# jjery2243542/adaptive_voice_conversion

Measured on NVIDIA H100. Metric: mel-segments/sec (80x128) train step, higher is better.
Workload: dtype tf32

## Files before the change

adaptive_voice_conversion_b200/csrc/wgrad_tc.cu:

```cuda
#include "common.cuh"
#include "tc_common.cuh"
#include "tmap.cuh"

namespace avc {

constexpr int WT_NT = 32;
constexpr int WG_ROWS = 32;
constexpr int WG_A_PLANE = 32 * 4 * 16;
constexpr int WG_A_BYTES = (WG_ROWS / 4) * WG_A_PLANE;
constexpr int WG_MAX_STAGES = 8;
constexpr int WG_SMEM_MAX = 224 * 1024;

struct WgTcArgs {
  avc_wgrad_desc d;
  float* scratch;
  int nslices, samp_per_slice, nstage, coutp;
  int* status;
};

__device__ __forceinline__ float comp4(const float4& v, int c) { return c == 0 ? v.x : c == 1 ? v.y : c == 2 ? v.z : v.w; }

struct WgJob {
  float4 v[4];
  uint32_t dst;
  int rot;
};

template <int K>
__device__ __forceinline__ WgJob wgrad_job_load(const WgTcArgs& a, int e, int ch, int b0, int R) {
  const avc_wgrad_desc& d = a.d;
  const int T = d.Tout;
  WgJob J;
  const int c4 = e & 7, pl = (e >> 3) & 7, j = e >> 6;
  const int r = ch * WG_ROWS + 4 * pl;
  const int g = r / T, t = r - g * T;
  J.rot = (c4 >> 1) & 3;
  J.dst = (uint32_t)WG_A_BYTES + (uint32_t)pl * (uint32_t)(K * WT_NT * 16) + (uint32_t)(j * WT_NT + 4 * c4) * 16u;
  const int ci = blockIdx.x * WT_NT + 4 * c4;
  const bool v = r < R && ci < d.Cin;
  const float* col = d.x + (size_t)(v ? b0 + g : 0) * d.x_bstride + (size_t)((v ? ci : 0) >> 2) * d.Tin * 4;
#pragma unroll
  for (int i = 0; i < 4; ++i) {
    const int p = src_pos((t + i) * d.stride + j - d.pad_left, d.Tin, AVC_PAD_REFLECT, 1);
    J.v[i] = (v && p >= 0) ? ldg4(col + (size_t)p * 4) : zero4();
  }
  return J;
}

__device__ __forceinline__ void wgrad_job_store(uint8_t* stage, const WgJob& J) {
#pragma unroll
  for (int k = 0; k < 4; ++k) {
    const int c = (k + J.rot) & 3;
    *reinterpret_cast<float4*>(stage + J.dst + (uint32_t)c * 16u) = make_float4(comp4(J.v[0], c), comp4(J.v[1], c), comp4(J.v[2], c), comp4(J.v[3], c));
  }
}

__host__ __device__ constexpr int wg_stagers(int K) { return K <= 6 ? 2 : 1; }
__host__ __device__ constexpr int wg_threads(int K) { return 128 * (wg_stagers(K) + 2); }
__host__ __device__ constexpr int wg_regs_stage(int K) { return wg_stagers(K) == 2 ? 96 : 104; }
__host__ __device__ constexpr int wg_regs_mma(int K) { return wg_stagers(K) == 2 ? 160 : 200; }
static_assert(2 * 128 * wg_regs_stage(1) + 256 * wg_regs_mma(1) <= 512 * 128 && 128 * wg_regs_stage(8) + 256 * wg_regs_mma(8) <= 384 * 168,
              "setmaxnreg budget exceeds the launch allocation");

template <int N>
__device__ __forceinline__ bool wgrad_mma_stage(const WgTcArgs& a, float* acc, uint32_t* af, uint32_t* af_prev, uint64_t* full, int s, uint32_t ph,
                                                const uint8_t* stage, uint32_t a_off, uint32_t b_lo, uint32_t d_hi) {
  constexpr uint32_t B_PLANE = N * 16;
  if (!__all_sync(0xffffffffu, tc::mbar_wait(&full[s], ph, a.status, 6))) {
    tc::wgmma_wait<0>();
    return false;
  }
#pragma unroll
  for (int k = 0; k < WG_ROWS / 8; ++k)
#pragma unroll
    for (int q = 0; q < 4; ++q)
      af[4 * k + q] = *reinterpret_cast<const uint32_t*>(stage + a_off + (uint32_t)(2 * k + (q >> 1)) * WG_A_PLANE + (uint32_t)(q & 1) * 128u);
  tc::wgmma_fence();
#pragma unroll
  for (int k = 0; k < WG_ROWS / 8; ++k)
    tc::wgmma_tf32_rs<N>(acc, af + 4 * k, tc::sdesc64(b_lo + (uint32_t)k * ((2u * B_PLANE) >> 4), d_hi), 1u);
  tc::wgmma_commit();
  tc::wgmma_wait<1>();
  tc::acc_fence(acc, N / 2);
  tc::reg_fence(af_prev, 16);
  return true;
}

template <int K, bool ATOMIC>
__global__ void __launch_bounds__(wg_threads(K), 1) conv_wgrad_wgmma_kernel(const WgTcArgs a, const __grid_constant__ CUtensorMap tmdc) {
  constexpr int STAGERS = wg_stagers(K);
  constexpr int N = K * WT_NT;
  constexpr uint32_t B_PLANE = N * 16;
  extern __shared__ __align__(1024) uint8_t smem[];
  __shared__ uint64_t bar_full[WG_MAX_STAGES], bar_empty[WG_MAX_STAGES];
  const avc_wgrad_desc& d = a.d;
  const int tid = threadIdx.x, warp = tc::warp_idx_sync(), lane = tid & 31;
  const int sl = blockIdx.z, b0 = sl * a.samp_per_slice;
  const int R = max(0, min(a.samp_per_slice, d.B - b0)) * d.Tout;
  const int nchunk = cdiv(R, WG_ROWS);
  const uint32_t stage_bytes = (uint32_t)WG_A_BYTES + 8u * B_PLANE;

  if (tid == 0) {
    for (int s = 0; s < a.nstage; ++s) {
      tc::mbar_init(&bar_full[s], 5);
      tc::mbar_init(&bar_empty[s], 2);
    }
    tc::fence_mbar_init();
  }
  __syncthreads();

  if (warp < 4 * STAGERS) {
    tc::setmaxnreg_dec<wg_regs_stage(K)>();
    constexpr int NJOBS = 64 * K, JPT = (NJOBS + 127) / 128;
    const int stid = tid & 127;
    for (int ch = warp >> 2; ch < nchunk; ch += STAGERS) {
      const int s = ch % a.nstage;
      const uint32_t ph = (uint32_t)(ch / a.nstage) & 1u;
      WgJob J[JPT];
#pragma unroll
      for (int q = 0; q < JPT; ++q)
        if (stid + 128 * q < NJOBS) J[q] = wgrad_job_load<K>(a, stid + 128 * q, ch, b0, R);
      if (ch >= a.nstage && !__all_sync(0xffffffffu, tc::mbar_wait(&bar_empty[s], ph ^ 1u, a.status, 5))) return;
      uint8_t* stage = smem + (size_t)s * stage_bytes;
      if (stid == 0) {
        tc::mbar_arrive_expect_tx(&bar_full[s], (uint32_t)WG_A_BYTES);
#pragma unroll
        for (int p = 0; p < WG_ROWS / 4; ++p) {
          const int r = ch * WG_ROWS + 4 * p, g = r / d.Tout;
          tc::tensor_g2s_4d(stage + p * WG_A_PLANE, &tmdc, 0, r - g * d.Tout, blockIdx.y * 32, r < R ? b0 + g : d.B, &bar_full[s]);
        }
      }
#pragma unroll
      for (int q = 0; q < JPT; ++q)
        if (stid + 128 * q < NJOBS) wgrad_job_store(stage, J[q]);
      tc::fence_proxy_async_smem();
      __syncwarp();
      if (lane == 0) tc::mbar_arrive(&bar_full[s]);
    }
    return;
  }

  tc::setmaxnreg_inc<wg_regs_mma(K)>();
  const int wg = (warp >> 2) - STAGERS, wt = tid & 127;
  float acc[N / 2];
#pragma unroll
  for (int i = 0; i < N / 2; ++i) acc[i] = 0.f;
  const int m = 64 * wg + tc::wg_acc_row(wt, 0);
  const uint32_t a_off = (uint32_t)(m >> 2) * 64u + (uint32_t)(wt & 3) * 16u + (uint32_t)(m & 3) * 4u;
  uint32_t af[2][16];
  const uint32_t smem0 = tc::smem_u32(smem), d_hi = tc::sdesc_hi(128);
  int s = 0, s_prev = -1;
  uint32_t ph = 0;
  tc::acc_fence(acc, N / 2);
  for (int ch = 0; ch < nchunk; ++ch) {
    const uint32_t b_lo = tc::sdesc_lo(smem0 + (uint32_t)s * stage_bytes + (uint32_t)WG_A_BYTES, B_PLANE);
    const uint8_t* stage = smem + (size_t)s * stage_bytes;
    const bool ok = (ch & 1) ? wgrad_mma_stage<N>(a, acc, af[1], af[0], bar_full, s, ph, stage, a_off, b_lo, d_hi)
                             : wgrad_mma_stage<N>(a, acc, af[0], af[1], bar_full, s, ph, stage, a_off, b_lo, d_hi);
    if (!ok) return;
    if (s_prev >= 0 && wt == 0) tc::mbar_arrive(&bar_empty[s_prev]);
    s_prev = s;
    if (++s == a.nstage) { s = 0; ph ^= 1u; }
  }
  tc::wgmma_wait<0>();
  tc::acc_fence(acc, N / 2);
  tc::reg_fence(af[0], 16);
  tc::reg_fence(af[1], 16);
  if (nchunk == 0) return;

  const int co = blockIdx.y * 128 + m;
#pragma unroll
  for (int jj = 0; jj < N / 8; ++jj) {
    const int n = tc::wg_acc_col(wt, 4 * jj), j = n / WT_NT, ci = blockIdx.x * WT_NT + n % WT_NT;
    if (ci < d.Cin) {
      float* sbase = a.scratch + (((size_t)(ATOMIC ? 0 : sl) * K + j) * (size_t)(d.Cin >> 2)) * (size_t)a.coutp * 4;
#pragma unroll
      for (int h = 0; h < 2; ++h) {
        float* p = sbase + ((size_t)(ci >> 2) * a.coutp + co + 8 * h) * 4 + (ci & 3);
        const float v0 = acc[4 * jj + 2 * h], v1 = acc[4 * jj + 2 * h + 1];
        if constexpr (ATOMIC)
          asm volatile("red.global.add.v2.f32 [%0], {%1, %2};" ::"l"(p), "f"(v0), "f"(v1) : "memory");
        else
          *reinterpret_cast<float2*>(p) = make_float2(v0, v1);
      }
    }
  }
}

__global__ void __launch_bounds__(256) wgrad_tc_reduce_kernel(const float* __restrict__ scratch, float* __restrict__ dw, int Cout, int Cin,
                                                              int K, int coutp, int nslices) {
  __shared__ float4 part[8][32];
  const int64_t n = (int64_t)K * (Cin >> 2) * coutp;
  const int64_t slice_stride = n * 4;
  const int64_t i = (int64_t)blockIdx.x * 32 + threadIdx.x;
  float4 s = zero4();
  if (i < n) {
    int sl = threadIdx.y;
    float4 s1 = zero4();
    const float* p = scratch + i * 4;
    for (; sl + 24 < nslices; sl += 32) {
      const float4 v0 = ldg4(p + (sl + 0) * slice_stride), v1 = ldg4(p + (sl + 8) * slice_stride);
      const float4 v2 = ldg4(p + (sl + 16) * slice_stride), v3 = ldg4(p + (sl + 24) * slice_stride);
      s.x += v0.x + v2.x; s.y += v0.y + v2.y; s.z += v0.z + v2.z; s.w += v0.w + v2.w;
      s1.x += v1.x + v3.x; s1.y += v1.y + v3.y; s1.z += v1.z + v3.z; s1.w += v1.w + v3.w;
    }
    s.x += s1.x; s.y += s1.y; s.z += s1.z; s.w += s1.w;
    for (; sl < nslices; sl += 8) {
      const float4 v = ldg4(scratch + sl * slice_stride + i * 4);
      s.x += v.x; s.y += v.y; s.z += v.z; s.w += v.w;
    }
  }
  part[threadIdx.y][threadIdx.x] = s;
  __syncthreads();
  if (threadIdx.y == 0 && i < n) {
#pragma unroll
    for (int y = 1; y < 8; ++y) { const float4 v = part[y][threadIdx.x]; s.x += v.x; s.y += v.y; s.z += v.z; s.w += v.w; }
    const int co = (int)(i % coutp);
    if (co < Cout) {
      const int64_t r = i / coutp;
      const int c4 = (int)(r % (Cin >> 2)), j = (int)(r / (Cin >> 2));
      float* o = dw + ((int64_t)co * Cin + c4 * 4) * K + j;
      o[0] += s.x; o[K] += s.y; o[2 * K] += s.z; o[3 * K] += s.w;
    }
  }
}

__global__ void __launch_bounds__(256) wgrad_acc_flush_kernel(const avc_wgrad_acc_item* __restrict__ items) {
  __shared__ float tile[32][32 * 8 + 1];
  const avc_wgrad_acc_item it = items[blockIdx.y];
  const int K = it.K, C4 = it.Cin >> 2;
  const int coutp = cdiv(it.Cout, 128) * 128;
  const int ncg = cdiv(C4, 8);
  const int nblk = (coutp >> 5) * ncg;
  if ((int)blockIdx.x >= nblk) return;
  const int cot = blockIdx.x / ncg, cg = blockIdx.x - cot * ncg;
  const int co0 = cot << 5, c40 = cg << 3;
  const int tid = threadIdx.x, col = tid & 31, c4l = tid >> 5;
  if (c40 + c4l < C4) {
    for (int j = 0; j < K; ++j) {
      float4* a4 = reinterpret_cast<float4*>(it.acc) + ((size_t)j * C4 + c40 + c4l) * coutp + co0 + col;
      const float4 s = *a4;
      *a4 = zero4();
      float* t = &tile[col][(c4l * 4) * K + j];
      t[0] = s.x; t[K] = s.y; t[2 * K] = s.z; t[3 * K] = s.w;
    }
  }
  __syncthreads();
  const int nci = min(32, it.Cin - c40 * 4);
  const int run = nci * K;
  for (int r = tid >> 5; r < 32; r += 8) {
    const int co = co0 + r;
    if (co >= it.Cout) break;
    float* o = it.dw + ((size_t)co * it.Cin + c40 * 4) * K;
    for (int e = tid & 31; e < run; e += 32) o[e] += tile[r][e];
  }
}

static int wgrad_tc_plan(const avc_wgrad_desc* d, WgTcArgs& a) {
  const int T = d->Tout;
  a.d = *d;
  int G = T >= 128 ? 1 : 128 / T;
  if (d->stride == 2) G = T >= 64 ? 1 : 64 / T;
  a.coutp = cdiv(d->Cout, 128) * 128;
  const int ntiles = cdiv(d->B, G);
  const int cta_per_slice = cdiv(d->Cin, WT_NT) * cdiv(d->Cout, 128);
  int nsl = 132 / cta_per_slice;
  if (nsl < 1) nsl = 1;
  if (nsl > ntiles) nsl = ntiles;
  const int tiles_per_slice = cdiv(ntiles, nsl);
  a.nslices = cdiv(ntiles, tiles_per_slice);
  a.samp_per_slice = tiles_per_slice * G;
  a.nstage = min(WG_MAX_STAGES, WG_SMEM_MAX / (WG_A_BYTES + 8 * 16 * WT_NT * d->K));
  return AVC_OK;
}

static bool wgrad_tc_supported(const avc_wgrad_desc* d) {
  return (d->stride == 1 || d->stride == 2) && d->Tout % 8 == 0 && d->Tout <= 128 && d->K >= 1 && d->K <= 8 && d->Cin % 4 == 0 &&
         d->Cout % 4 == 0 && d->Tin + d->K - 1 >= (d->Tout - 1) * d->stride + 1 && (d->stride == 1 || d->Tout <= 64);
}

int wgrad_reduce(const float* scratch, float* dw, int Cout, int Cin, int K, int coutp, int nslices, cudaStream_t stream) {
  const int64_t n = (int64_t)K * (Cin / 4) * coutp;
  AVC_LAUNCH(wgrad_tc_reduce_kernel, (int)cdiv64(n, 32), dim3(32, 8), 0, stream, scratch, dw, Cout, Cin, K, coutp, nslices);
  AVC_CHECK_LAUNCH("wgrad_tc_reduce");
  return AVC_OK;
}

template <int K, bool ATOMIC>
static int wgrad_wgmma_launch(const WgTcArgs& a, const CUtensorMap& tmdc, cudaStream_t stream, const char* who) {
  static bool attr_done = false;
  if (!attr_done) {
    const cudaError_t e = cudaFuncSetAttribute(conv_wgrad_wgmma_kernel<K, ATOMIC>, cudaFuncAttributeMaxDynamicSharedMemorySize, WG_SMEM_MAX);
    if (e != cudaSuccess) {
      set_error("%s: cudaFuncSetAttribute: %s", who, cudaGetErrorString(e));
      return AVC_ERR_CUDA;
    }
    attr_done = true;
  }
  const dim3 grid(cdiv(a.d.Cin, WT_NT), cdiv(a.d.Cout, 128), a.nslices);
  const int smem = a.nstage * (WG_A_BYTES + 8 * 16 * WT_NT * K);
  AVC_LAUNCH((conv_wgrad_wgmma_kernel<K, ATOMIC>), grid, wg_threads(K), smem, stream, a, tmdc);
  AVC_CHECK_LAUNCH(who);
  return AVC_OK;
}

template <bool ATOMIC>
static int wgrad_wgmma_dispatch(const WgTcArgs& a, const CUtensorMap& tmdc, cudaStream_t stream, const char* who) {
  switch (a.d.K) {
    case 1: return wgrad_wgmma_launch<1, ATOMIC>(a, tmdc, stream, who);
    case 2: return wgrad_wgmma_launch<2, ATOMIC>(a, tmdc, stream, who);
    case 3: return wgrad_wgmma_launch<3, ATOMIC>(a, tmdc, stream, who);
    case 4: return wgrad_wgmma_launch<4, ATOMIC>(a, tmdc, stream, who);
    case 5: return wgrad_wgmma_launch<5, ATOMIC>(a, tmdc, stream, who);
    case 6: return wgrad_wgmma_launch<6, ATOMIC>(a, tmdc, stream, who);
    case 7: return wgrad_wgmma_launch<7, ATOMIC>(a, tmdc, stream, who);
    default: return wgrad_wgmma_launch<8, ATOMIC>(a, tmdc, stream, who);
  }
}

}

using namespace avc;

extern "C" int64_t avc_wgrad_tc_scratch_floats(const avc_wgrad_desc* d) {
  if (!d || !wgrad_tc_supported(d)) return -1;
  WgTcArgs a;
  wgrad_tc_plan(d, a);
  return (int64_t)a.nslices * d->K * d->Cin * a.coutp;
}

static int wgrad_tc_launch(const avc_wgrad_desc* d, float* scratch, int* status, void* stream, bool accumulate, const char* who) {
  AVC_REQUIRE(d && d->x && d->dc && scratch && status && (accumulate || d->dw), AVC_ERR_INVALID, "%s: null argument", who);
  AVC_REQUIRE(d->B > 0 && d->Cin > 0 && d->Cout > 0 && d->Tin > 0 && d->Tout > 0, AVC_ERR_INVALID, "%s: bad shape", who);
  AVC_REQUIRE(wgrad_tc_supported(d), AVC_ERR_UNSUPPORTED, "%s: needs stride 1 (Tout <= 128) or 2 (Tout <= 64), Tout %% 8 == 0, K <= 8", who);
  AVC_REQUIRE(((uintptr_t)d->dc & 15u) == 0 && d->dc_bstride % 4 == 0, AVC_ERR_UNSUPPORTED,
              "%s: dc and its sample stride (%lld floats) must be 16-byte aligned", who, (long long)d->dc_bstride);
  WgTcArgs a;
  wgrad_tc_plan(d, a);
  a.scratch = scratch;
  a.status = status;
  CUtensorMap tmdc;
  {
    PFN_tmap_encode enc = tmap_encode_fn();
    AVC_REQUIRE(enc, AVC_ERR_CUDA, "%s: cuTensorMapEncodeTiled is not available from this driver", who);
    const cuuint64_t gdim[4] = {4, (cuuint64_t)d->Tout, (cuuint64_t)(d->Cout / 4), (cuuint64_t)d->B};
    const cuuint64_t gstr[3] = {16, (cuuint64_t)d->Tout * 16u, (cuuint64_t)d->dc_bstride * 4u};
    const cuuint32_t box[4] = {4, 4, 32, 1};
    const cuuint32_t estr[4] = {1, 1, 1, 1};
    const CUresult r = enc(&tmdc, CU_TENSOR_MAP_DATA_TYPE_FLOAT32, 4, (void*)d->dc, gdim, gstr, box, estr, CU_TENSOR_MAP_INTERLEAVE_NONE,
                           CU_TENSOR_MAP_SWIZZLE_NONE, CU_TENSOR_MAP_L2_PROMOTION_L2_256B, CU_TENSOR_MAP_FLOAT_OOB_FILL_NONE);
    AVC_REQUIRE(r == CUDA_SUCCESS, AVC_ERR_CUDA, "%s: cuTensorMapEncodeTiled failed (%d) for dc: B=%d Cout=%d Tout=%d bstride=%lld", who, (int)r,
                d->B, d->Cout, d->Tout, (long long)d->dc_bstride);
  }
  const int rc = accumulate ? wgrad_wgmma_dispatch<true>(a, tmdc, (cudaStream_t)stream, who)
                            : wgrad_wgmma_dispatch<false>(a, tmdc, (cudaStream_t)stream, who);
  if (rc != AVC_OK || accumulate) return rc;
  return wgrad_reduce(scratch, d->dw, d->Cout, d->Cin, d->K, a.coutp, a.nslices, (cudaStream_t)stream);
}

extern "C" int avc_conv_wgrad_tc(const avc_wgrad_desc* d, float* scratch, int* status, void* stream) {
  return wgrad_tc_launch(d, scratch, status, stream, false, "avc_conv_wgrad_tc");
}

extern "C" int64_t avc_wgrad_acc_floats(int Cout, int Cin, int K) {
  if (Cout <= 0 || Cin <= 0 || K <= 0 || Cin % 4 != 0) return -1;
  return (int64_t)K * Cin * (cdiv(Cout, 128) * 128);
}
extern "C" int avc_conv_wgrad_tc_acc(const avc_wgrad_desc* d, float* acc, int* status, void* stream) {
  return wgrad_tc_launch(d, acc, status, stream, true, "avc_conv_wgrad_tc_acc");
}
extern "C" int avc_wgrad_acc_flush(const avc_wgrad_acc_item* items_dev, int n_items, int64_t max_units, void* stream) {
  AVC_REQUIRE(items_dev && n_items > 0 && max_units > 0, AVC_ERR_INVALID, "avc_wgrad_acc_flush: bad argument");
  dim3 grid((unsigned)cdiv64(max_units, 256) + 64u, (unsigned)n_items);
  AVC_LAUNCH(wgrad_acc_flush_kernel, grid, 256, 0, (cudaStream_t)stream, items_dev);
  AVC_CHECK_LAUNCH("wgrad_acc_flush");
  return AVC_OK;
}
```

Measured before the change: 36140.

## Stage wgrad input windows per thread with load reuse and half-group prefetch

Replaces the per-(tap,row) staging jobs with per-thread sliding windows: each thread loads 3*S+K contiguous float4 units once and emits all K taps from registers, so overlapping input positions are no longer reloaded for every tap. The stager warpgroups are split into 64-thread halves that each own a chunk, and when the register budget allows, the next chunk's window is loaded before the current one is stored. The full-barrier arrival count and the setmaxnreg splits are adjusted to match. The cost is more staging registers, a separate fast path for in-bounds windows, and a stricter ring-depth assumption that is checked by static_asserts.

```diff
diff --git a/adaptive_voice_conversion_b200/csrc/wgrad_tc.cu b/adaptive_voice_conversion_b200/csrc/wgrad_tc.cu
--- a/adaptive_voice_conversion_b200/csrc/wgrad_tc.cu
+++ b/adaptive_voice_conversion_b200/csrc/wgrad_tc.cu
@@ -18,49 +18,113 @@
   int* status;
 };
 
-__device__ __forceinline__ float comp4(const float4& v, int c) { return c == 0 ? v.x : c == 1 ? v.y : c == 2 ? v.z : v.w; }
-
-struct WgJob {
-  float4 v[4];
-  uint32_t dst;
-  int rot;
-};
-
-template <int K>
-__device__ __forceinline__ WgJob wgrad_job_load(const WgTcArgs& a, int e, int ch, int b0, int R) {
+__host__ __device__ constexpr int wg_win_units(int K, int S) { return 3 * S + K; }
+
+template <int K, int S>
+__device__ __forceinline__ void wgrad_win_load(const WgTcArgs& a, float4 (&u)[wg_win_units(K, S)], int w, int ch, int b0, int R) {
   const avc_wgrad_desc& d = a.d;
-  const int T = d.Tout;
-  WgJob J;
-  const int c4 = e & 7, pl = (e >> 3) & 7, j = e >> 6;
+  const int c4 = w & 7, pl = w >> 3;
   const int r = ch * WG_ROWS + 4 * pl;
-  const int g = r / T, t = r - g * T;
-  J.rot = (c4 >> 1) & 3;
-  J.dst = (uint32_t)WG_A_BYTES + (uint32_t)pl * (uint32_t)(K * WT_NT * 16) + (uint32_t)(j * WT_NT + 4 * c4) * 16u;
+  const int g = r / d.Tout, t = r - g * d.Tout;
   const int ci = blockIdx.x * WT_NT + 4 * c4;
   const bool v = r < R && ci < d.Cin;
   const float* col = d.x + (size_t)(v ? b0 + g : 0) * d.x_bstride + (size_t)((v ? ci : 0) >> 2) * d.Tin * 4;
-#pragma unroll
-  for (int i = 0; i < 4; ++i) {
-    const int p = src_pos((t + i) * d.stride + j - d.pad_left, d.Tin, AVC_PAD_REFLECT, 1);
-    J.v[i] = (v && p >= 0) ? ldg4(col + (size_t)p * 4) : zero4();
-  }
-  return J;
-}
-
-__device__ __forceinline__ void wgrad_job_store(uint8_t* stage, const WgJob& J) {
+  const int p0 = t * S - d.pad_left;
+  if (v && p0 >= 0 && p0 + wg_win_units(K, S) <= d.Tin) {
+    const float* q = col + (size_t)p0 * 4;
+#pragma unroll
+    for (int n = 0; n < wg_win_units(K, S); ++n) u[n] = ldg4(q + 4 * n);
+  } else {
+#pragma unroll
+    for (int n = 0; n < wg_win_units(K, S); ++n) {
+      const int p = src_pos(p0 + n, d.Tin, AVC_PAD_REFLECT, 1);
+      u[n] = (v && p >= 0) ? ldg4(col + (size_t)p * 4) : zero4();
+    }
+  }
+}
+
+__device__ __forceinline__ float comp4(const float4& v, int c) { return c == 0 ? v.x : c == 1 ? v.y : c == 2 ? v.z : v.w; }
+__device__ __forceinline__ float4 rot4(float4 v, int rot) {
+  if (rot & 1) v = make_float4(v.y, v.z, v.w, v.x);
+  if (rot & 2) v = make_float4(v.z, v.w, v.x, v.y);
+  return v;
+}
+
+template <int K, int S>
+__device__ __forceinline__ void wgrad_win_store(uint8_t* stage, float4 (&u)[wg_win_units(K, S)], int w) {
+  const int c4 = w & 7, pl = w >> 3, rot = (c4 >> 1) & 3;
+  uint8_t* row = stage + WG_A_BYTES + pl * (K * WT_NT * 16) + c4 * 64;
+#pragma unroll
+  for (int n = 0; n < wg_win_units(K, S); ++n) u[n] = rot4(u[n], rot);
 #pragma unroll
   for (int k = 0; k < 4; ++k) {
-    const int c = (k + J.rot) & 3;
-    *reinterpret_cast<float4*>(stage + J.dst + (uint32_t)c * 16u) = make_float4(comp4(J.v[0], c), comp4(J.v[1], c), comp4(J.v[2], c), comp4(J.v[3], c));
+    uint8_t* dst = row + ((k + rot) & 3) * 16;
+#pragma unroll
+    for (int j = 0; j < K; ++j)
+      *reinterpret_cast<float4*>(dst + j * WT_NT * 16) = make_float4(comp4(u[j], k), comp4(u[S + j], k), comp4(u[2 * S + j], k), comp4(u[3 * S + j], k));
   }
 }
 
 __host__ __device__ constexpr int wg_stagers(int K) { return K <= 6 ? 2 : 1; }
+__host__ __device__ constexpr int wg_halves(int K) { return 2 * wg_stagers(K); }
 __host__ __device__ constexpr int wg_threads(int K) { return 128 * (wg_stagers(K) + 2); }
-__host__ __device__ constexpr int wg_regs_stage(int K) { return wg_stagers(K) == 2 ? 96 : 104; }
-__host__ __device__ constexpr int wg_regs_mma(int K) { return wg_stagers(K) == 2 ? 160 : 200; }
-static_assert(2 * 128 * wg_regs_stage(1) + 256 * wg_regs_mma(1) <= 512 * 128 && 128 * wg_regs_stage(8) + 256 * wg_regs_mma(8) <= 384 * 168,
-              "setmaxnreg budget exceeds the launch allocation");
+__host__ __device__ constexpr int wg_regs_stage(int K) { return K <= 4 ? 128 : K == 5 ? 112 : K == 6 ? 96 : 120; }
+__host__ __device__ constexpr int wg_regs_mma(int K) { return K <= 4 ? 128 : K == 5 ? 144 : K == 6 ? 160 : 192; }
+__host__ __device__ constexpr bool wg_prefetch(int K, int S) { return 2 * 4 * wg_win_units(K, S) + 40 <= wg_regs_stage(K); }
+__host__ __device__ constexpr bool wg_budget_ok(int K) {
+  return K > 8 || (wg_stagers(K) * 128 * wg_regs_stage(K) + 256 * wg_regs_mma(K) <= wg_threads(K) * (wg_stagers(K) == 2 ? 128 : 168) &&
+                   wg_budget_ok(K + 1));
+}
+static_assert(wg_budget_ok(1), "setmaxnreg budget exceeds the launch allocation");
+__host__ __device__ constexpr bool wg_ring_ok(int K) {
+  return K > 8 || ((WG_SMEM_MAX / (WG_A_BYTES + 8 * 16 * WT_NT * K) >= wg_halves(K)) && wg_ring_ok(K + 1));
+}
+static_assert(wg_ring_ok(1), "a staging half could run a whole ring ahead");
+
+template <int K, int S>
+__device__ __forceinline__ bool wgrad_win_put(const WgTcArgs& a, const CUtensorMap* tmdc, uint8_t* smem, uint64_t* full, uint64_t* empty,
+                                              float4 (&u)[wg_win_units(K, S)], int w, int ch, int b0, int R) {
+  const avc_wgrad_desc& d = a.d;
+  const int s = ch % a.nstage;
+  const uint32_t ph = (uint32_t)(ch / a.nstage) & 1u;
+  if (ch >= a.nstage && !__all_sync(0xffffffffu, tc::mbar_wait(&empty[s], ph ^ 1u, a.status, 5))) return false;
+  uint8_t* stage = smem + (size_t)s * ((uint32_t)WG_A_BYTES + 8u * (uint32_t)(K * WT_NT * 16));
+  if (w == 0) {
+    tc::mbar_arrive_expect_tx(&full[s], (uint32_t)WG_A_BYTES);
+#pragma unroll
+    for (int p = 0; p < WG_ROWS / 4; ++p) {
+      const int r = ch * WG_ROWS + 4 * p, g = r / d.Tout;
+      tc::tensor_g2s_4d(stage + p * WG_A_PLANE, tmdc, 0, r - g * d.Tout, blockIdx.y * 32, r < R ? b0 + g : d.B, &full[s]);
+    }
+  }
+  wgrad_win_store<K, S>(stage, u, w);
+  tc::fence_proxy_async_smem();
+  __syncwarp();
+  if ((w & 31) == 0) tc::mbar_arrive(&full[s]);
+  return true;
+}
+
+template <int K, int S>
+__device__ __forceinline__ void wgrad_stage_x(const WgTcArgs& a, const CUtensorMap* tmdc, uint8_t* smem, uint64_t* full, uint64_t* empty,
+                                              int h, int w, int b0, int R, int nchunk) {
+  constexpr int H = wg_halves(K), U = wg_win_units(K, S);
+  float4 ua[U];
+  if constexpr (wg_prefetch(K, S)) {
+    float4 ub[U];
+    if (h < nchunk) wgrad_win_load<K, S>(a, ua, w, h, b0, R);
+    for (int ch = h; ch < nchunk; ch += 2 * H) {
+      if (ch + H < nchunk) wgrad_win_load<K, S>(a, ub, w, ch + H, b0, R);
+      if (!wgrad_win_put<K, S>(a, tmdc, smem, full, empty, ua, w, ch, b0, R) || ch + H >= nchunk) return;
+      if (ch + 2 * H < nchunk) wgrad_win_load<K, S>(a, ua, w, ch + 2 * H, b0, R);
+      if (!wgrad_win_put<K, S>(a, tmdc, smem, full, empty, ub, w, ch + H, b0, R)) return;
+    }
+  } else {
+    for (int ch = h; ch < nchunk; ch += H) {
+      wgrad_win_load<K, S>(a, ua, w, ch, b0, R);
+      if (!wgrad_win_put<K, S>(a, tmdc, smem, full, empty, ua, w, ch, b0, R)) return;
+    }
+  }
+}
 
 template <int N>
 __device__ __forceinline__ bool wgrad_mma_stage(const WgTcArgs& a, float* acc, uint32_t* af, uint32_t* af_prev, uint64_t* full, int s, uint32_t ph,
@@ -94,7 +158,7 @@
   extern __shared__ __align__(1024) uint8_t smem[];
   __shared__ uint64_t bar_full[WG_MAX_STAGES], bar_empty[WG_MAX_STAGES];
   const avc_wgrad_desc& d = a.d;
-  const int tid = threadIdx.x, warp = tc::warp_idx_sync(), lane = tid & 31;
+  const int tid = threadIdx.x, warp = tc::warp_idx_sync();
   const int sl = blockIdx.z, b0 = sl * a.samp_per_slice;
   const int R = max(0, min(a.samp_per_slice, d.B - b0)) * d.Tout;
   const int nchunk = cdiv(R, WG_ROWS);
@@ -102,7 +166,7 @@
 
   if (tid == 0) {
     for (int s = 0; s < a.nstage; ++s) {
-      tc::mbar_init(&bar_full[s], 5);
+      tc::mbar_init(&bar_full[s], 3);
       tc::mbar_init(&bar_empty[s], 2);
     }
     tc::fence_mbar_init();
@@ -111,32 +175,10 @@
 
   if (warp < 4 * STAGERS) {
     tc::setmaxnreg_dec<wg_regs_stage(K)>();
-    constexpr int NJOBS = 64 * K, JPT = (NJOBS + 127) / 128;
-    const int stid = tid & 127;
-    for (int ch = warp >> 2; ch < nchunk; ch += STAGERS) {
-      const int s = ch % a.nstage;
-      const uint32_t ph = (uint32_t)(ch / a.nstage) & 1u;
-      WgJob J[JPT];
-#pragma unroll
-      for (int q = 0; q < JPT; ++q)
-        if (stid + 128 * q < NJOBS) J[q] = wgrad_job_load<K>(a, stid + 128 * q, ch, b0, R);
-      if (ch >= a.nstage && !__all_sync(0xffffffffu, tc::mbar_wait(&bar_empty[s], ph ^ 1u, a.status, 5))) return;
-      uint8_t* stage = smem + (size_t)s * stage_bytes;
-      if (stid == 0) {
-        tc::mbar_arrive_expect_tx(&bar_full[s], (uint32_t)WG_A_BYTES);
-#pragma unroll
-        for (int p = 0; p < WG_ROWS / 4; ++p) {
-          const int r = ch * WG_ROWS + 4 * p, g = r / d.Tout;
-          tc::tensor_g2s_4d(stage + p * WG_A_PLANE, &tmdc, 0, r - g * d.Tout, blockIdx.y * 32, r < R ? b0 + g : d.B, &bar_full[s]);
-        }
-      }
-#pragma unroll
-      for (int q = 0; q < JPT; ++q)
-        if (stid + 128 * q < NJOBS) wgrad_job_store(stage, J[q]);
-      tc::fence_proxy_async_smem();
-      __syncwarp();
-      if (lane == 0) tc::mbar_arrive(&bar_full[s]);
-    }
+    if (d.stride == 1)
+      wgrad_stage_x<K, 1>(a, &tmdc, smem, bar_full, bar_empty, warp >> 1, tid & 63, b0, R, nchunk);
+    else
+      wgrad_stage_x<K, 2>(a, &tmdc, smem, bar_full, bar_empty, warp >> 1, tid & 63, b0, R, nchunk);
     return;
   }
 
```

After: 38190, median of 6. 5.7% higher.
